# Kolkir/feature-point-cnn

Measured on AMD Instinct MI355X. Metric: frames/sec (VGA 640x480) SuperPoint fwd+NMS+descriptors, higher is better.
Workload: dtype f32

## Files before the change

feature-point-cnn_amd/_lib.py:

```python
import ctypes
import os
import subprocess

import torch

_DIR = os.path.dirname(os.path.abspath(__file__))
LIB_PATH = os.environ.get("FPC_LIB_PATH") or os.path.join(_DIR, "lib", "libfpc.so")
CSRC = os.path.join(_DIR, "csrc")

SYMBOLS = [
    "fpc_abi_version", "fpc_build_flags", "fpc_strerror", "fpc_last_hip_error", "fpc_default_config", "fpc_create",
    "fpc_destroy", "fpc_load_weights", "fpc_packed_size", "fpc_packed_device_ptr",
    "fpc_export_packed", "fpc_import_packed", "fpc_import_packed_device", "fpc_mark_weights_loaded", "fpc_set_stream", "fpc_upload_stream",
    "fpc_get_stream", "fpc_sync", "fpc_forward", "fpc_detect", "fpc_get_points", "fpc_results",
    "fpc_get_counts", "fpc_get_keypoints", "fpc_set_timing", "fpc_get_timings", "fpc_match", "fpc_first_within",
    "fpc_detect_u8", "fpc_u8_staging", "fpc_homography_adaptation", "fpc_detect_u8_resized",
    "fpc_sample_descriptors", "fpc_plan_hash", "fpc_broadcast_weights", "fpc_read_activation",
    "fpc_pack_layout_revision", "fpc_tile_choice", "fpc_check_guards", "fpc_stream_report", "fpc_output_range",
    "fpc_match_frames", "fpc_first_within_frames",
    "fpc_default_ransac_params", "fpc_ransac_homography", "fpc_homography_frames",
    "fpc_bank_create", "fpc_bank_destroy", "fpc_bank_get", "fpc_bank_store", "fpc_bank_store_rows", "fpc_bank_clear",
    "fpc_match_bank", "fpc_homography_bank", "fpc_bank_create_ex", "fpc_bank_format",
    "fpc_match_frames_guided", "fpc_match_bank_guided",
    "fpc_cell_order", "fpc_match_frames_guided_cells", "fpc_match_bank_guided_cells",
    "fpc_bank_topk_reserve", "fpc_match_bank_topk", "fpc_homography_bank_topk",
    "fpc_ransac_fundamental", "fpc_fundamental_frames", "fpc_fundamental_bank",
    "fpc_match_frames_guided_epipolar", "fpc_match_bank_guided_epipolar",
    "fpc_match_frames_guided_epipolar_cells", "fpc_match_bank_guided_epipolar_cells",
    "fpc_default_pose_params", "fpc_pose_fundamental", "fpc_pose_frames", "fpc_pose_bank",
    "fpc_default_pnp_params", "fpc_pnp_reserve", "fpc_bank_landmarks_reserve", "fpc_bank_store_landmarks",
    "fpc_bank_landmarks_get", "fpc_ransac_pnp", "fpc_pnp_frames", "fpc_pnp_bank",
]

ABI_VERSION = 4
PACK_LAYOUT_REVISION = 4

PLAN_FLAGS = {
    "no_fused_blocks": 1 << 0, "no_winograd": 1 << 1, "no_winograd_detector": 1 << 2, "no_winograd_layer_in1": 1 << 3,
    "no_xcd_order": 1 << 4, "no_fused_stem_pool": 1 << 5, "split_heads": 1 << 6, "nms_in_line": 1 << 7,
    "no_persistent_grid": 1 << 8, "layer1_tile_8x16": 1 << 9, "winograd_gen1": 1 << 10, "no_latency_tiles": 1 << 11,
    "nms_one_workgroup": 1 << 12, "no_fused_softmax": 1 << 13, "winograd_gen2": 1 << 14, "guard_zones": 1 << 15, "detector_gen1": 1 << 16, "heads_in_line": 1 << 17, "w36_one_wave": 1 << 18, "convt_phases": 1 << 19, "stem_round3": 1 << 20, "conv_round1": 1 << 21,
    "tiles_round5": 1 << 22,
}


class FpcConfig(ctypes.Structure):
    _fields_ = [("device", ctypes.c_int), ("height", ctypes.c_int), ("width", ctypes.c_int),
                ("max_batch", ctypes.c_int), ("cell", ctypes.c_int), ("nms_dist", ctypes.c_int),
                ("conf_thresh", ctypes.c_float), ("border_remove", ctypes.c_int),
                ("descriptor_enabled", ctypes.c_int), ("max_keypoints", ctypes.c_int),
                ("in_channels", ctypes.c_int), ("dtype", ctypes.c_int), ("arch", ctypes.c_int),
                ("num_streams", ctypes.c_int), ("plan_flags", ctypes.c_uint), ("nms_round_launches", ctypes.c_int),
                ("min_sub_batch", ctypes.c_int)]


class FpcTensor(ctypes.Structure):
    _fields_ = [("name", ctypes.c_char_p), ("data", ctypes.c_void_p), ("ndim", ctypes.c_int),
                ("shape", ctypes.c_int64 * 4)]


class FpcDeviceResults(ctypes.Structure):
    _fields_ = [("count", ctypes.c_void_p), ("n_candidates", ctypes.c_void_p), ("xy", ctypes.c_void_p),
                ("conf", ctypes.c_void_p), ("desc", ctypes.c_void_p), ("capacity", ctypes.c_int),
                ("desc_dim", ctypes.c_int)]


class FpcStreamReport(ctypes.Structure):
    _fields_ = [("n_streams", ctypes.c_int), ("slot", ctypes.c_int * 16), ("queue", ctypes.c_int * 16),
                ("probing", ctypes.c_int), ("hw_queues_found", ctypes.c_int), ("process_probe_rounds", ctypes.c_int),
                ("process_probe_launches", ctypes.c_int), ("process_inconclusive_rounds", ctypes.c_int),
                ("process_probe_ms", ctypes.c_float), ("create_probe_rounds", ctypes.c_int),
                ("create_placement_ms", ctypes.c_float), ("process_registered_streams", ctypes.c_int)]


class FpcRansacParams(ctypes.Structure):
# ... 170 lines not shown
```

feature-point-cnn_amd/csrc/block_mfma.h:

```cpp
#pragma once
#include "conv_mfma.h"

namespace fpc {

#ifdef FPC_DIAG
#define FPC_STAMP(i)                                                                     \
  if (a.stamps && threadIdx.x == 0) {                                                    \
    unsigned long long t_;                                                               \
    asm volatile("s_memtime %0\n\ts_waitcnt lgkmcnt(0)" : "=s"(t_)::"memory");            \
    a.stamps[(size_t)blockIdx.x * 8 + (i)] = t_;                                         \
  }
#define FPC_RSTAMP(i)                                                                    \
  if (a.stamps && threadIdx.x == 0) {                                                    \
    unsigned long long t_;                                                               \
    asm volatile("s_memrealtime %0\n\ts_waitcnt lgkmcnt(0)" : "=s"(t_)::"memory");        \
    a.stamps[(size_t)blockIdx.x * 8 + (i)] = t_;                                         \
  }
#else
#define FPC_STAMP(i)
#define FPC_RSTAMP(i)
#endif

struct BlockArgs {
  const float* x;
  int csx, nchunk;
  int H, W;
  const float4* w1;
  const float* b1;
  int tapoff4[9];
  const float4* w2;
  const float* b2;
  int k8_h, k8_x;
  float* out;
  int cso, Ho, Wo, tiles_x, tiles_y, nstore, frame0;
  unsigned x_bytes;
#ifdef FPC_DIAG
  unsigned long long* stamps;
#endif
};

template <int TH, int TW, int S, int KC, int WM, int WN, int MB, int NB, int CMIDP>
struct BlockCfg {
  using C1 = ConvCfg<TH, TW, S, 3, KC, WM, WN, MB, NB>;
  static constexpr int ROWH4 = CMIDP / 4 + 1;
  static constexpr int H_BYTES = C1::M * ROWH4 * 16;
  static constexpr int LDS_BYTES = C1::LDS_BYTES > H_BYTES ? C1::LDS_BYTES : H_BYTES;
  static_assert(CMIDP % 8 == 0 && CMIDP <= C1::N, "mid channels must fit the workgroup's N");
};

template <int TH, int TW, int S, int KC, int WM, int WN, int MB, int NB, int CMIDP>
__global__ __launch_bounds__(WM* WN * 64, 2) void block_mfma_kernel(const BlockArgs a) {
  using C = ConvCfg<TH, TW, S, 3, KC, WM, WN, MB, NB>;
  using BC = BlockCfg<TH, TW, S, KC, WM, WN, MB, NB, CMIDP>;
  constexpr int NT = C::NT, HW = C::HW, HH = C::HH, ROW4 = C::ROW4, K8 = KC / 8, KC4 = KC / 4;
  constexpr int NV = HH * HW * KC4, ITER = (NV + NT - 1) / NT, ROWH4 = BC::ROWH4, NBT = WN * NB;
  extern __shared__ float4 lds4[];

  const int tid = threadIdx.x, lane = tid & 63, wave = tid >> 6;
  const int wm = wave / WN, wn = wave % WN;
  const int half = lane >> 5, l31 = lane & 31;
  const int tiles = a.tiles_x * a.tiles_y;
  const int bidx = fpc_xcd_tile_index();
  const int bl = bidx / tiles;
  const int b = a.frame0 + bl;
  const int t = bidx - bl * tiles;
  const int ty = t / a.tiles_x, tx = t - ty * a.tiles_x;

  FPC_STAMP(0)
#ifdef FPC_DIAG
  if (a.stamps && threadIdx.x == 0) {
    a.stamps[(size_t)blockIdx.x * 8 + 6] = __builtin_amdgcn_s_getreg(63492);
    a.stamps[(size_t)blockIdx.x * 8 + 7] = __builtin_amdgcn_s_getreg((31 << 11) | 20);
  }
#endif
  int abase[MB];
#pragma unroll
  for (int mb = 0; mb < MB; ++mb) {
    int m = (wm * MB + mb) * 32 + l31;
    m = m < TH * TW ? m : TH * TW - 1;
    const int py = m / TW, px = m - py * TW;
    abase[mb] = ((py * S) * HW + px * S) * ROW4 + half;
  }
  constexpr int stepstride = NBT * 64;
  const __amdgpu_buffer_rsrc_t wrsrc = __builtin_amdgcn_make_buffer_rsrc(
      const_cast<float4*>(a.w1), 0, (int)((unsigned)(a.nchunk * 9 * K8 + 2) * (unsigned)(stepstride * 16)), 0x00020000);
  const int wlane = ((wn * NB) * 64 + lane) * 16;
  int wstep = 0;
  auto wfrag = [&](int nb) {
    typedef float f32x4w __attribute__((ext_vector_type(4)));
    const f32x4w r = __builtin_bit_cast(f32x4w, __builtin_amdgcn_raw_buffer_load_b128(wrsrc, wlane + nb * 1024, wstep, 0));
    return make_float4(r.x, r.y, r.z, r.w);
  };

  const int iy0 = ty * TH * S - 1, ix0 = tx * TW * S - 1;
  typedef float f32x4v __attribute__((ext_vector_type(4)));
  f32x4v stage[ITER];
  const __amdgpu_buffer_rsrc_t xrsrc = __builtin_amdgcn_make_buffer_rsrc(const_cast<float*>(a.x), 0, (int)a.x_bytes, 0x00020000);
  const unsigned xbase = (unsigned)((b * a.H + iy0) * a.W + ix0) * (unsigned)(a.csx * 4);
  auto load_chunk = [&](int chunk) {
    const int wlim = chunk < a.nchunk ? a.W : 0;
#pragma unroll
    for (int i = 0; i < ITER; ++i) {
      const int e = tid + i * NT;
      const int pix = e / KC4, c4 = e - pix * KC4;
      const int hy = pix / HW, hx = pix - hy * HW;
      const int iy = iy0 + hy, ix = ix0 + hx;
      const bool ok = ((unsigned)iy < (unsigned)a.H) & ((unsigned)ix < (unsigned)wlim) & (hy < HH);
      unsigned off = xbase + (unsigned)(((hy * a.W + hx) * a.csx + chunk * KC + c4 * 4) * 4);
      asm volatile("" : "+v"(off));
      stage[i] = __builtin_bit_cast(f32x4v, __builtin_amdgcn_raw_buffer_load_b128(xrsrc, (int)(ok ? off : 0xfffffff0u), 0, 0));
    }
  };
  auto store_chunk = [&]() {
#pragma unroll
    for (int i = 0; i < ITER; ++i) {
      const int e = tid + i * NT;
      int pix = e / KC4, c4 = e - pix * KC4;
      if (NV % NT != 0) {
        const bool in = e < NV;
        pix = in ? pix : HH * HW - 1;
        c4 = in ? c4 : KC4;
      }
      *reinterpret_cast<f32x4v*>(&lds4[pix * ROW4 + c4]) = stage[i];
    }
  };

  f32x16 acc[MB][NB];
#pragma unroll
  for (int mb = 0; mb < MB; ++mb)
#pragma unroll
    for (int nb = 0; nb < NB; ++nb)
#pragma unroll
      for (int r = 0; r < 16; ++r) acc[mb][nb][r] = 0.f;

  load_chunk(0);
  float4 b0[NB], b1[NB];
#pragma unroll
  for (int nb = 0; nb < NB; ++nb) b0[nb] = wfrag(nb);
  wstep += stepstride * 16;
#pragma unroll
// ... 181 lines not shown
        const int e = tid + i * NT;
        const int m = e / C4, c4 = e - m * C4;
        const int py = m / TW, px = m - py * TW;
        const int y = oyb + py, x = oxb + px;
        const bool ok = (NE % NT == 0 || e < NE) && y < a.Ho && x < a.Wo;
        idv[i] = *reinterpret_cast<const float4*>(a.x + (ok ? ((size_t)(b * a.Ho + y) * a.Wo + x) * a.csx + c4 * 4 : 0));
      }
    }
#pragma unroll
    for (int i = 0; i < EIT; ++i) {
      const int e = tid + i * NT;
      const int m = e / C4, c4 = e - m * C4;
      const int py = m / TW, px = m - py * TW;
      const int y = oyb + py, x = oxb + px;
      if ((NE % NT == 0 || e < NE) && y < a.Ho && x < a.Wo) {
        float4 v = lds4[m * ROWH4 + c4];
        if (ident) {
          v.x += idv[i].x;
          v.y += idv[i].y;
          v.z += idv[i].z;
          v.w += idv[i].w;
        }
        v.x = v.x > 0.f ? v.x : 0.f;
        v.y = v.y > 0.f ? v.y : 0.f;
        v.z = v.z > 0.f ? v.z : 0.f;
        v.w = v.w > 0.f ? v.w : 0.f;
        *reinterpret_cast<float4*>(a.out + ((size_t)(b * a.Ho + y) * a.Wo + x) * a.cso + c4 * 4) = v;
      }
    }
  }
  FPC_STAMP(5)
}


}
```

feature-point-cnn_amd/csrc/fpc_api.hip:

```cpp
#include <hip/hip_runtime.h>

#include <dlfcn.h>

#include <algorithm>
#include <cmath>
#include <cstdio>
#include <cstdlib>
#include <cstring>
#include <memory>
#include <mutex>
#include <chrono>
#include <string>
#include <vector>

#include "../../include/fpc.h"
#include "block_mfma.h"
#include "block_bf16.h"
#include "convt_bf16.h"
#include "block_x3.h"
#include "stem_bf16.h"
#include "wblock_mfma.h"
#include "wblock16_mfma.h"
#include "wblock36_mfma.h"
#include "wblock36p_mfma.h"
// ... 126 lines not shown
enum BKind {
#define X(name, ...) BK_##name,
  FPC_BLOCK_KINDS(X)
#undef X
      BK_COUNT
};

struct BKindInfo {
  const char* name;
  const char* symbol;
  int TH, TW, S, KC, WM, WN, MB, NB, CMIDP;
  int lds_bytes;
  const void* fn;
  void (*launch)(const BlockArgs&, dim3, hipStream_t);
};

#define X(name, TH, TW, S, KC, WM, WN, MB, NB, CMIDP)                                                     \
  static void launchb_##name(const BlockArgs& a, dim3 grid, hipStream_t st) {                             \
    using BC = BlockCfg<TH, TW, S, KC, WM, WN, MB, NB, CMIDP>;                                            \
    hipLaunchKernelGGL((block_mfma_kernel<TH, TW, S, KC, WM, WN, MB, NB, CMIDP>), grid, dim3(WM* WN * 64), \
                       BC::LDS_BYTES, st, a);                                                             \
  }
FPC_BLOCK_KINDS(X)
#undef X

static const BKindInfo g_bkinds[BK_COUNT] = {
#define X(name, TH, TW, S, KC, WM, WN, MB, NB, CMIDP)                                                      \
  {#name, "block_mfma_kernel<" #TH ", " #TW ", " #S ", " #KC ", " #WM ", " #WN ", " #MB ", " #NB ", " #CMIDP ">", \
   TH, TW, S, KC, WM, WN, MB, NB, CMIDP, BlockCfg<TH, TW, S, KC, WM, WN, MB, NB, CMIDP>::LDS_BYTES,         \
   (const void*)block_mfma_kernel<TH, TW, S, KC, WM, WN, MB, NB, CMIDP>, launchb_##name},
    FPC_BLOCK_KINDS(X)
#undef X
};

#define FPC_WBLOCK_KINDS(X)     \
  X(W816_K32_C64, 32, 2, 64)    \
  X(W816_K32_C128, 32, 4, 128)  \
  X(W816_K32_C72, 32, 3, 72)    \
  X(W816_K24_C72, 24, 3, 72)
#define FPC_W16_KINDS(X) \
  X(W16_C64, 4, 8)       \
  X(W16_C128, 8, 8)      \
  X(W16_C128H, 8, 4)
#define FPC_W36_KINDS(X) \
  X(W36_C64_4x4, 1, 4, 4)  \
  X(W36_C64_2x8, 1, 2, 8)  \
  X(W36_C128_4x4, 2, 4, 4) \
  X(W36_C128_2x8, 2, 2, 8)

#define FPC_W36P_KINDS(X) \
  X(W36P_C64_4x4, 4, 4)   \
  X(W36P_C64_2x8, 2, 8)

#define FPC_W36PD_KINDS(X) \
  X(W36PD_C65_4x4, 4, 4)   \
  X(W36PD_C65_2x8, 2, 8)

#define FPC_W36D_KINDS(X) \
  X(W36_C65_4x4, 4, 4)    \
  X(W36_C65_2x8, 2, 8)

#define FPC_W36S_KINDS(X) \
  X(W36S_C128_4x4, 2, 4, 4)
#define FPC_W36PC_KINDS(X) \
  X(W36PC_C64_8x2, 8, 2)

// ... 243 lines not shown
  BlockArgs bargs{};
  WKind wkind = WK_COUNT;
  int hash_bkind = -1, hash_wkind = -1;
  WBlockArgs wargs{};
  FKind fkind = FK_COUNT;
  BlockBfArgs fargs{};
  int phase = -1;
  int when = 0;
  bool shadow = false;
  bool wconv = false;
  int n0 = 0;
  bool plain_conv = false;
  bool lean = false;
  int ksize = 0;
  const float* pin = nullptr;
  float* pout = nullptr;
  int pH = 0, pW = 0, pC = 0;
  std::string prefix;
  int cin = 0, cout = 0;
  int grid_y = 1, grid_z = 1;
  double flops_per_frame = 0;
  double mfma_flops_per_frame = 0;
  bool fused_softmax_capable = false;
  double bytes_per_frame = 0;
  bool descriptor_branch = false;
};

struct Timing {
  hipEvent_t start, stop;
  int op;
  int frames;
  int wkind = -1;
  double mfma_flops = -1.0;
};

}

using namespace fpc;

struct fpc_ctx {
  fpc_config cfg{};
  int H = 0, W = 0, B = 0, Hc = 0, Wc = 0;
  bool vgg = false;
  int D = 128;
  std::vector<float*> vbuf;
  size_t vconv0_off = 0;
  bool bf16 = false;
  bool split = false;
  bool split_f16 = false;
  int lgcs = 72;
  int cin = 3;
  int cap = 0, sort_cap = 0;
  hipStream_t stream = nullptr;
  bool own_stream = false;
  hipStream_t upload = nullptr;
  bool queue_probe = true;
  int probe_rounds = 0;
  double placement_ms = 0.0;
  std::vector<std::pair<hipStream_t, int>> caller_stream_memo;
  std::vector<hipStream_t> aux;
  std::vector<hipEvent_t> ev_join;
  std::vector<hipStream_t> side;
  std::vector<hipEvent_t> ev_enc, ev_det;
  bool nms_aside = true;
  bool split_heads = false;
  hipEvent_t ev_fork = nullptr;
  int min_sub = 8;
  int num_cus = 256;
  int fkind_blocks_per_cu[64] = {};
  int persist_min_tiles = 1;
  bool xcd_order = true;
  int nms_passes = 2;
  bool fuse_softmax = true;
  bool convt_fused = true;
  bool logits_valid = false;
  bool nms_one_workgroup = false;
  int nms_g = 0;
  bool fuse_stem_pool = true;
  bool conv_lean = true;
  bool stem_lean = true;
  bool stem2 = false;
  bool layer1_t816 = false;
#ifdef FPC_DIAG
  unsigned long long* diag_stamps = nullptr;
  int diag_n = 0;
#endif
  bool winograd_in1 = true;
  bool winograd_det = true;
  int w36_cus = 0;
  bool tiles_round6 = true;
  bool w36_paired = true;
  bool winograd_det_gen3 = true;
  bool winograd = true;
  bool latency_tiles = true;
  int winograd_gen = 3;
  bool fuse_blocks = true;
  bool weights_loaded = false;
  bool plan_error = false;

  char* slab = nullptr;
  size_t slab_bytes = 0;
  bool guard_zones = false;
  std::vector<std::pair<size_t, size_t>> guards;
  float *stem_out, *x0, *h4, *x1, *x2, *h8, *x3, *cat, *dh, *dproj, *d0, *lg;
  float *h16, *y16a, *y16b, *lo_h, *lo0, *desc_map, *desc_in_nhwc;
  float* prob;
  uint32_t *nmsmap, *cand;
  int32_t *ncand, *count, *xy, *status;
  float* rowmax = nullptr;
  uint32_t* range = nullptr;
  float *conf, *desc_out;
  unsigned long long* sort_scratch;
  int32_t* nms_aux = nullptr;
  unsigned long long *rowbest, *colbest;
  float* mf_norms = nullptr;
  unsigned long long *mf_top2 = nullptr, *mf_colbest = nullptr;
  float4* hf_pairs = nullptr;
  int32_t *hf_row = nullptr, *hf_np = nullptr;
  unsigned long long* hf_best = nullptr;
  int32_t *mgc_perm_q = nullptr, *mgc_perm_t = nullptr;
  int4* mgc_box = nullptr;
  char* bank_slab = nullptr;
// ... 1671 lines not shown
      default: break;
    }
    if (rc != FPC_OK) return rc;
  }
  return FPC_OK;
}

static hipEvent_t next_event(fpc_ctx* c) {
  if (c->events_used == c->event_pool.size()) {
    hipEvent_t e;
    hipEventCreate(&e);
    c->event_pool.push_back(e);
  }
  return c->event_pool[c->events_used++];
}

struct Sub {
  int f0, n;
  bool small = false;
  bool fuse_softmax = false;
  hipStream_t st;
  hipStream_t side = nullptr;
  hipEvent_t ev_enc = nullptr, ev_det = nullptr;
};

struct LaunchTimer {
  fpc_ctx* c;
  int op;
  hipStream_t st;
  int frames;
  hipEvent_t s{}, e{};
  int wkind = -1;
  double mfma_flops = -1.0;
  LaunchTimer(fpc_ctx* c_, int op_, hipStream_t st_, int frames_) : c(c_), op(op_), st(st_), frames(frames_) {
    if (c->timing) {
      s = next_event(c);
      e = next_event(c);
      hipEventRecord(s, st);
    }
  }
  ~LaunchTimer() {
    if (c->timing) {
      hipEventRecord(e, st);
      c->timings.push_back({s, e, op, frames, wkind, mfma_flops});
    }
  }
};

static int op_index(const fpc_ctx* c, OpType t) {
  for (size_t i = 0; i < c->ops.size(); ++i)
    if (c->ops[i].type == t) return (int)i;
  return -1;
}

template <typename Args>
static void diag_stamp(fpc_ctx* c, const Op& op, Args& a, int tiles) {
#ifdef FPC_DIAG
  a.stamps = nullptr;
  if (const char* e = getenv("FPC_STAMP_OP"))
    if (op.name.find(e) != std::string::npos) {
      if (!c->diag_stamps) hipHostMalloc((void**)&c->diag_stamps, (size_t)65536 * 8 * sizeof(unsigned long long));
      memset(c->diag_stamps, 0, (size_t)65536 * 8 * sizeof(unsigned long long));
      a.stamps = c->diag_stamps;
      c->diag_n = tiles;
    }
#endif
}

enum StemKind { STEM_PLAIN, STEM_POOL, STEM_POOL2, STEM_X3, STEM_X3_F16, STEM_BF16 };
static StemKind stem_kind(const fpc_ctx* c) {
  if (!(c->fuse_stem_pool || c->cin == 1 || c->bf16)) return STEM_PLAIN;
  if (c->split_f16) return STEM_X3_F16;
  if (c->bf16) return STEM_BF16;
  if (c->split) return STEM_X3;
  return c->stem2 ? STEM_POOL2 : STEM_POOL;
}

// ... 89 lines not shown
    const WKind sk = c->tiles_round6 ? w36_stacked_kind(op.wkind) : WK_COUNT;
    double mf = 0.0;
    for (int g0 = 0; g0 < n; g0 += fpl) {
      const int gn = std::min(fpl, n - g0);
      a.frame0 = 0;
      a.x = x0 + (size_t)(f0 + g0) * Hf * a.W * a.csx;
      a.out = o0 + (size_t)(f0 + g0) * Hf * a.W * a.cso;
      a.x_bytes = (unsigned)((unsigned long long)gn * Hf * a.W * a.csx * sizeof(float));
      const int srows = w36_stacked_rows(Hf, a.W, gn, sk, tx_f * ty_f);
      const WKind lk = srows ? sk : op.wkind;
      a.H = srows ? gn * Hf : Hf;
      a.frame_h = srows ? Hf : 0;
      a.tiles_x = srows ? (a.W + g_wkinds[sk].TW - 1) / g_wkinds[sk].TW : tx_f;
      a.tiles_y = srows ? srows : ty_f;
      a.total = srows ? a.tiles_x * srows : tx_f * ty_f * gn;
      if (srows) t.wkind = sk;
      mf += srows ? wkind_mfma_flops(g_wkinds[sk], a.total, a.nchunk, a.k8_h + a.k8_x) : op.mfma_flops_per_frame * gn;
      const int cus_cap = c->w36_cus > 0 ? std::min(c->num_cus, c->w36_cus) : c->num_cus;
      const int cus8 = std::max(1, cus_cap / 8 / std::max(1, op.grid_y)), per_xcd = (a.total + 7) / 8;
      const int rounds = (per_xcd + cus8 - 1) / cus8;
      const int grid3 = 8 * std::min(cus8, (per_xcd + rounds - 1) / rounds);
      g_wkinds[lk].launch(a, dim3(std::min(a.total, grid3), op.grid_y), sb.st);
    }
    if (t.wkind >= 0) t.mfma_flops = mf;
    return;
  }
  g_wkinds[op.wkind].launch(a, dim3(std::min(a.total, grid), op.grid_y), sb.st);
}

static void launch_block(fpc_ctx* c, const Op& op, int i, const Sub& sb) {
  LaunchTimer t(c, i, sb.st, sb.n);
  BlockArgs a = op.bargs;
  a.frame0 = sb.f0;
  diag_stamp(c, op, a, a.tiles_x * a.tiles_y * sb.n);
  g_bkinds[op.bkind].launch(a, dim3(a.tiles_x * a.tiles_y * sb.n), sb.st);
}

static void launch_fblock(fpc_ctx* c, const Op& op, int i, const Sub& sb) {
  const int n = sb.n, f0 = sb.f0;
  LaunchTimer t(c, i, sb.st, n);
  BlockBfArgs a = op.fargs;
  a.frame0 = f0;
  a.range_flag = c->split_f16 ? c->status + 1 : nullptr;
  diag_stamp(c, op, a, a.tiles_x * a.tiles_y * n);
  if (g_fkinds[op.fkind].planes != 1) {
    g_fkinds[op.fkind].launch(a, dim3(a.tiles_x * a.tiles_y * n), sb.st);
    return;
  }
  a.total_tiles = a.tiles_x * a.tiles_y * n;
  if (sb.fuse_softmax && op.fused_softmax_capable) {
    const size_t HW = (size_t)c->H * c->W;
    hipMemsetAsync(c->ncand + f0, 0, sizeof(int32_t) * n, sb.st);
    a.softmax = 1;
    a.thresh = c->cfg.conf_thresh;
    a.nmsmap = c->nmsmap + f0 * HW;
    a.cand = c->cand + f0 * HW;
    a.ncand = c->ncand + f0;
  }
  const int g = std::min((a.total_tiles + 7) / 8 * 8, std::max(8, c->fkind_blocks_per_cu[op.fkind] * c->num_cus / op.grid_y / 8 * 8));
  g_fkinds[op.fkind].launch(a, dim3(g, op.grid_y), sb.st);
}

static void launch_conv(fpc_ctx* c, const Op& op, int i, const Sub& sb) {
  LaunchTimer t(c, i, sb.st, sb.n);
  ConvArgs a = op.args;
  a.frame0 = sb.f0;
// ... 222 lines not shown
    case FPC_E_MISSING_KEY: return "checkpoint entry missing or of the wrong shape (see fpc_last_hip_error)";
    case FPC_E_CAPACITY: return "caller buffer too small";
    case FPC_E_NOT_CONVERGED: return "NMS round limit hit";
    case FPC_E_RANGE: return "value outside fp16's range in FPC_F32_SPLIT_F16 mode (use FPC_F32_SPLIT or FPC_F32)";
    case FPC_E_NONFINITE: return "a frame of the call holds a NaN or Inf pixel (see fpc_last_hip_error for which)";
    default: return "unknown error";
  }
}

const char* fpc_last_hip_error(void) { return g_hip_err.c_str(); }

int fpc_default_config(fpc_config* cfg) {
  if (!cfg) return FPC_E_INVALID;
  memset(cfg, 0, sizeof(*cfg));
  cfg->device = 0;
  cfg->height = 480;
  cfg->width = 640;
  cfg->max_batch = 1;
  cfg->cell = 8;
  cfg->nms_dist = 4;
  cfg->conf_thresh = 0.015f;
  cfg->border_remove = 4;
  cfg->descriptor_enabled = 1;
  cfg->max_keypoints = 0;
  return FPC_OK;
}

enum { SLOT_MAIN = 0, SLOT_AUX = 1, SLOT_SIDE = 100, SLOT_UPLOAD = 200 };

static int prepare_kernels(fpc_ctx* c, const fpc_config* cfg) {
  for (int k = 0; k < K_COUNT; ++k)
    HIPCHECK(hipFuncSetAttribute(g_kinds[k].fn, hipFuncAttributeMaxDynamicSharedMemorySize, g_kinds[k].lds_bytes));
  for (const LeanKindInfo& l : g_lean_kinds) HIPCHECK(hipFuncSetAttribute(l.fn, hipFuncAttributeMaxDynamicSharedMemorySize, l.lds_bytes));
  for (int k = 0; k < WK_COUNT; ++k)
    HIPCHECK(hipFuncSetAttribute(g_wkinds[k].fn, hipFuncAttributeMaxDynamicSharedMemorySize, g_wkinds[k].lds_bytes));
  for (int k = 0; k < BK_COUNT; ++k)
    HIPCHECK(hipFuncSetAttribute(g_bkinds[k].fn, hipFuncAttributeMaxDynamicSharedMemorySize, g_bkinds[k].lds_bytes));
  static_assert(FK_COUNT <= 64, "fpc_ctx::fkind_blocks_per_cu");
  for (int k = 0; k < FK_COUNT; ++k) {
    HIPCHECK(hipFuncSetAttribute(g_fkinds[k].fn, hipFuncAttributeMaxDynamicSharedMemorySize, g_fkinds[k].lds_bytes));
    int nb = 0;
    HIPCHECK(hipOccupancyMaxActiveBlocksPerMultiprocessor(&nb, g_fkinds[k].fn, g_fkinds[k].WM * g_fkinds[k].WN * 64, g_fkinds[k].lds_bytes));
    c->fkind_blocks_per_cu[k] = std::max(1, nb);
#ifdef FPC_DIAG
    hipFuncAttributes fa{};
    hipFuncGetAttributes(&fa, g_fkinds[k].fn);
    fprintf(stderr, "[diag] %s: lds %d B, regs %d, scratch %zu, occupancy %d blocks/CU\n", g_fkinds[k].name, g_fkinds[k].lds_bytes, fa.numRegs, fa.localSizeBytes, nb);
#endif
  }
  HIPCHECK(hipFuncSetAttribute((const void*)softmax_d2s_kernel<false>, hipFuncAttributeMaxDynamicSharedMemorySize,
                               12 * cfg->width * (int)sizeof(float)));
  HIPCHECK(hipFuncSetAttribute((const void*)softmax_d2s_kernel<true>, hipFuncAttributeMaxDynamicSharedMemorySize,
                               12 * cfg->width * (int)sizeof(float)));
  HIPCHECK(hipFuncSetAttribute((const void*)stem_bf16_kernel<1>, hipFuncAttributeMaxDynamicSharedMemorySize, StemB2Cfg<1>::LDS_BYTES));
  HIPCHECK(hipFuncSetAttribute((const void*)stem_bf16_kernel<3>, hipFuncAttributeMaxDynamicSharedMemorySize, StemB2Cfg<3>::LDS_BYTES));
  HIPCHECK(hipFuncSetAttribute((const void*)nms_sort_kernel, hipFuncAttributeMaxDynamicSharedMemorySize,
                               NMS_LDS_KEYS * (int)sizeof(unsigned long long)));
#ifdef FPC_DIAG
  for (int k = 0; k < BK_COUNT; ++k) {
    int nb = -1;
    hipOccupancyMaxActiveBlocksPerMultiprocessor(&nb, g_bkinds[k].fn, g_bkinds[k].WM * g_bkinds[k].WN * 64, g_bkinds[k].lds_bytes);
    hipFuncAttributes fa{};
    hipFuncGetAttributes(&fa, g_bkinds[k].fn);
    fprintf(stderr, "[diag] %s: lds %d B, regs %d, static lds %zu, occupancy %d blocks/CU\n", g_bkinds[k].name, g_bkinds[k].lds_bytes, fa.numRegs, fa.sharedSizeBytes, nb);
  }
  for (int k = 0; k < K_COUNT; ++k) {
// ... 43 lines not shown
  c->D = c->vgg ? 256 : 128;
  c->bf16 = cfg->dtype == FPC_BF16;
  c->split = cfg->dtype == FPC_F32_SPLIT || cfg->dtype == FPC_F32_SPLIT_F16;
  c->split_f16 = cfg->dtype == FPC_F32_SPLIT_F16;
  c->lgcs = (c->bf16 || c->split) ? 80 : 72;
  const int r1 = cfg->nms_dist + 1;
  const int worst = ((c->H + r1 - 1) / r1) * ((c->W + r1 - 1) / r1);
  c->cap = cfg->max_keypoints > 0 ? cfg->max_keypoints : worst;
  c->sort_cap = 1;
  while (c->sort_cap < worst) c->sort_cap <<= 1;
  {
    const int prc = prepare_kernels(c.get(), cfg);
    if (prc != FPC_OK) return prc;
  }
  const bool qprobe = qmap::probe_mode() != 0;
  c->queue_probe = qprobe;
  const auto create_t0 = std::chrono::steady_clock::now();
  std::unique_lock<std::mutex> queue_lock(qmap::state().mu);
  const int probe_rounds0 = qmap::state().dev[cfg->device].rounds;
  c->stream = qmap::acquire(cfg->device, c.get(), SLOT_MAIN, true, qprobe, true);
  if (!c->stream) { qmap::release_owner(c.get()); g_hip_err = "hipStreamCreateWithFlags"; return FPC_E_HIP; }
  c->own_stream = true;
  {
    int nsub = cfg->num_streams > 0 ? std::min(8, cfg->num_streams) : (c->split ? 3 : 2);
    const unsigned pf = cfg->plan_flags;
    c->fuse_blocks = !(pf & FPC_PLAN_NO_FUSED_BLOCKS);
    c->guard_zones = (pf & FPC_PLAN_GUARD_ZONES) != 0;
    if (const char* e = getenv("FPC_GUARD_ZONES")) c->guard_zones = atoi(e) != 0;
    c->winograd_det_gen3 = !(pf & FPC_PLAN_DETECTOR_GEN1);
    c->w36_paired = !(pf & FPC_PLAN_W36_ONE_WAVE);
    if (const char* e = getenv("FPC_W36_PAIRED")) c->w36_paired = atoi(e) != 0;
    c->tiles_round6 = !(pf & FPC_PLAN_TILES_ROUND5);
    if (const char* e = getenv("FPC_TILES_ROUND6")) c->tiles_round6 = atoi(e) != 0;
    if (const char* e = getenv("FPC_W36_CUS")) c->w36_cus = std::max(0, atoi(e));
    if (const char* e = getenv("FPC_WINOGRAD_DET_GEN")) c->winograd_det_gen3 = atoi(e) >= 3;
    c->winograd = !(pf & FPC_PLAN_NO_WINOGRAD);
    c->winograd_det = !(pf & FPC_PLAN_NO_WINOGRAD_DETECTOR);
    c->winograd_in1 = !(pf & FPC_PLAN_NO_WINOGRAD_LAYER_IN1);
    c->xcd_order = !(pf & FPC_PLAN_NO_XCD_ORDER);
    c->fuse_stem_pool = !(pf & FPC_PLAN_NO_FUSED_STEM_POOL);
    c->stem_lean = !(pf & FPC_PLAN_STEM_ROUND3);
    c->conv_lean = !(pf & FPC_PLAN_CONV_ROUND1);
    if (const char* e = getenv("FPC_CONV_LEAN")) c->conv_lean = atoi(e) != 0;
    if (const char* e = getenv("FPC_STEM_LEAN")) c->stem_lean = atoi(e) != 0;
    c->split_heads = (pf & FPC_PLAN_SPLIT_HEADS) != 0;
    if (pf & FPC_PLAN_NO_PERSISTENT_GRID) c->persist_min_tiles = 0;
    c->layer1_t816 = (pf & FPC_PLAN_LAYER1_TILE_8x16) != 0;
    c->winograd_gen = (pf & FPC_PLAN_WINOGRAD_GEN1) ? 1 : (pf & FPC_PLAN_WINOGRAD_GEN2) ? 2 : 3;
    if (const char* e = getenv("FPC_WINOGRAD_GEN")) c->winograd_gen = std::min(3, std::max(1, atoi(e)));
    c->latency_tiles = !(pf & FPC_PLAN_NO_LATENCY_TILES);
    if (const char* e = getenv("FPC_LATENCY_TILES")) c->latency_tiles = atoi(e) != 0;
    c->fuse_softmax = !(pf & FPC_PLAN_NO_FUSED_SOFTMAX);
    c->convt_fused = !(pf & FPC_PLAN_CONVT_PHASES);
    if (const char* e = getenv("FPC_CONVT_FUSED")) c->convt_fused = atoi(e) != 0;
    if (const char* e = getenv("FPC_FUSE_SOFTMAX")) c->fuse_softmax = atoi(e) != 0;
    c->nms_one_workgroup = (pf & FPC_PLAN_NMS_ONE_WORKGROUP) != 0;
    if (const char* e = getenv("FPC_NMS_CHUNKED")) c->nms_one_workgroup = atoi(e) == 0;
    if (cfg->min_sub_batch > 0) c->min_sub = cfg->min_sub_batch;
    if (cfg->nms_round_launches > 0) c->nms_passes = std::min(64, cfg->nms_round_launches);
    else if (cfg->nms_round_launches < 0) c->nms_passes = 0;
    if (const char* e = getenv("FPC_STREAMS")) nsub = std::max(1, std::min(8, atoi(e)));
    if (!(pf & FPC_PLAN_HEADS_IN_LINE) && nsub >= 2 && !c->vgg && !c->bf16 && !c->split) c->split_heads = true;
    if (const char* e = getenv("FPC_FUSE")) c->fuse_blocks = atoi(e) != 0;
    if (const char* e = getenv("FPC_WINOGRAD")) c->winograd = atoi(e) != 0;
    if (const char* e = getenv("FPC_XCD_ORDER")) c->xcd_order = atoi(e) != 0;
    if (const char* e = getenv("FPC_MIN_SUB")) c->min_sub = std::max(1, atoi(e));
// ... 146 lines not shown
  if (n != c->blob_floats * sizeof(float)) {
    g_hip_err = "packed weights: " + std::to_string(n) + " bytes, this context's plan packs " + std::to_string(c->blob_floats * sizeof(float));
    return FPC_E_INVALID;
  }
  HIPCHECK(hipSetDevice(c->cfg.device));
  uint32_t h[BLOB_HEADER_FLOATS];
  HIPCHECK(hipMemcpy(h, src_dev, sizeof(h), hipMemcpyDeviceToHost));
  if (!check_blob_header(c, h, &g_hip_err)) return FPC_E_INVALID;
  if (src_dev != (const void*)c->blob) {
    c->weights_loaded = false;
    HIPCHECK(hipMemcpy(c->blob, src_dev, n, hipMemcpyDeviceToDevice));
    HIPCHECK(hipDeviceSynchronize());
  }
  c->weights_loaded = true;
  return FPC_OK;
}

int fpc_mark_weights_loaded(fpc_ctx* c) {
  if (!c) return FPC_E_INVALID;
  uint32_t h[BLOB_HEADER_FLOATS];
  HIPCHECK(hipSetDevice(c->cfg.device));
  HIPCHECK(hipMemcpy(h, c->blob, sizeof(h), hipMemcpyDeviceToHost));
  if (!check_blob_header(c, h, &g_hip_err)) {
    c->weights_loaded = false;
    return FPC_E_INVALID;
  }
  c->weights_loaded = true;
  return FPC_OK;
}

uint64_t fpc_plan_hash(const fpc_ctx* c) { return c ? plan_hash(c) : 0; }

int fpc_tile_choice(int what, int H, int W, int frames, unsigned plan_flags) {
  const bool r6 = !(plan_flags & FPC_PLAN_TILES_ROUND5);
  if (H <= 0 || W <= 0 || frames <= 0) return FPC_E_INVALID;
  switch (what) {
    case 0: {
      const WKindInfo& k = g_wkinds[w36_kind(128, H, W)];
      return r6 ? w36_stacked_rows(H, W, frames, WK_W36S_C128_4x4, ((H + k.TH - 1) / k.TH) * ((W + k.TW - 1) / k.TW)) : 0;
    }
    case 1: { const WKindInfo& k = g_wkinds[w36_kind(64, H, W, true, r6)]; return 100 * k.TH + k.TW; }
    case 2: {
      const BKind k5 = BK_B320_s2_K32_C128, k6 = BK_B416_s2_K32_C128;
      const BKindInfo& k = g_bkinds[r6 && block_rows(k6, H, W) < block_rows(k5, H, W) ? k6 : k5];
      return 100 * k.TH + k.TW;
    }
  }
  return FPC_E_INVALID;
}

int fpc_check_guards(fpc_ctx* c, long long* bad_words) {
  if (!c || !bad_words) return FPC_E_INVALID;
  *bad_words = 0;
  if (!c->guard_zones || c->guards.empty()) return FPC_E_INVALID;
  HIPCHECK(hipSetDevice(c->cfg.device));
  HIPCHECK(hipDeviceSynchronize());
  unsigned long long* d = nullptr;
  HIPCHECK(hipMalloc((void**)&d, sizeof(*d)));
  {
    const hipError_t e0 = hipMemset(d, 0, sizeof(*d));
    if (e0 != hipSuccess) hipFree(d);
    HIPCHECK(e0);
  }
  count_zones(c, c->slab, c->guards, d);
  count_zones(c, c->bank_slab, c->bank_guards, d);
  count_zones(c, c->topk_slab, c->topk_guards, d);
  count_zones(c, c->pnp_slab, c->pnp_guards, d);
  count_zones(c, c->lm_slab, c->lm_guards, d);
  unsigned long long h = 0;
  const hipError_t e1 = hipStreamSynchronize(c->stream);
  const hipError_t e2 = hipMemcpy(&h, d, sizeof(h), hipMemcpyDeviceToHost);
  hipFree(d);
  HIPCHECK(e1);
  HIPCHECK(e2);
  *bad_words = (long long)h;
  return FPC_OK;
}

namespace {
// ... 1320 lines not shown
  if (desc) {
    if (!c->cfg.descriptor_enabled) return FPC_E_INVALID;
    HIPCHECK(hipMemcpy(desc, c->desc_out + (size_t)frame * c->cap * c->D, sizeof(float) * c->D * k, hipMemcpyDeviceToHost));
  }
  return k;
}

int fpc_set_timing(fpc_ctx* c, int enable) {
  if (!c) return FPC_E_INVALID;
  c->timing_every = enable > 0 ? enable : 0;
  c->timing_calls = 0;
  c->timing = enable != 0;
  c->timings.clear();
  c->events_used = 0;
  return FPC_OK;
}

int fpc_get_timings(fpc_ctx* c, int cap, const char** names, const char** kernels, float* ms, double* flops,
                    double* mfma_flops, double* bytes) {
  if (!c) return FPC_E_INVALID;
  const int n = (int)c->timings.size();
  for (int i = 0; i < n && i < cap; ++i) {
    const Timing& t = c->timings[i];
    float v = 0.f;
    if (hipEventElapsedTime(&v, t.start, t.stop) != hipSuccess) v = -1.f;
    const Op* op = t.op >= 0 ? &c->ops[t.op] : nullptr;
    if (names) names[i] = op ? op->name.c_str() : "?";
    if (kernels) {
      const char* k = "?";
      if (op) switch (op->type) {
          case OP_STEM: k = launch_stem(c, *op, t.op, nullptr, nullptr); break;
          case OP_POOL: k = "maxpool_kernel"; break;
          case OP_CONV: k = op->lean ? lean_kind(op->kind)->symbol : g_kinds[op->kind].symbol; break;
          case OP_BLOCK: k = g_bkinds[op->bkind].symbol; break;
          case OP_WBLOCK: k = g_wkinds[t.wkind >= 0 ? t.wkind : op->wkind].symbol; break;
          case OP_BF16: k = g_fkinds[op->fkind].symbol; break;
          case OP_SOFTMAX: k = "softmax_d2s_kernel"; break;
          case OP_NMS: k = c->nms_one_workgroup ? "nms_rounds_kernel+nms_sort_kernel" : "nms_rounds_kernel+nms_finish_kernel+nms_chunk_sort_kernel+nms_merge_kernel"; break;
          case OP_DESC: k = "descriptor16_kernel"; break;
          case OP_VCONV0: k = "vgg_conv0_kernel"; break;
          case OP_POOL2: k = "maxpool2_kernel"; break;
          case OP_L2NORM: k = "l2norm256_kernel"; break;
        }
      kernels[i] = k;
    }
    if (ms) ms[i] = v;
    if (flops) flops[i] = op ? op->flops_per_frame * t.frames : 0.0;
    if (mfma_flops) mfma_flops[i] = !op ? 0.0 : t.mfma_flops >= 0 ? t.mfma_flops : op->mfma_flops_per_frame * t.frames;
    if (bytes) bytes[i] = op ? op->bytes_per_frame * t.frames : 0.0;
  }
  return n;
}

}
```

include/fpc.h:

```cpp
#ifndef FPC_H
#define FPC_H

#include <stddef.h>
#include <stdint.h>

#ifdef __cplusplus
extern "C" {
#endif

#define FPC_ABI_VERSION 4
#define FPC_PACK_LAYOUT_REVISION 4

enum {
  FPC_OK = 0,
  FPC_E_INVALID = -1,
  FPC_E_NO_DEVICE = -2,
  FPC_E_HIP = -3,
  FPC_E_NO_WEIGHTS = -4,
  FPC_E_MISSING_KEY = -5,
  FPC_E_CAPACITY = -6,
  FPC_E_NOT_CONVERGED = -7,
  FPC_E_RANGE = -8,
  FPC_E_NONFINITE = -9
};
// ... 14 lines not shown
  int max_keypoints;
  int in_channels;
  int dtype;
  int arch;
  int num_streams;
  unsigned plan_flags;
  int nms_round_launches;
  int min_sub_batch;
} fpc_config;

enum {
  FPC_PLAN_NO_FUSED_BLOCKS = 1 << 0,
  FPC_PLAN_NO_WINOGRAD = 1 << 1,
  FPC_PLAN_NO_WINOGRAD_DETECTOR = 1 << 2,
  FPC_PLAN_NO_WINOGRAD_LAYER_IN1 = 1 << 3,
  FPC_PLAN_NO_XCD_ORDER = 1 << 4,
  FPC_PLAN_NO_FUSED_STEM_POOL = 1 << 5,
  FPC_PLAN_SPLIT_HEADS = 1 << 6,
  FPC_PLAN_NMS_IN_LINE = 1 << 7,
  FPC_PLAN_NO_PERSISTENT_GRID = 1 << 8,
  FPC_PLAN_LAYER1_TILE_8x16 = 1 << 9,
  FPC_PLAN_WINOGRAD_GEN1 = 1 << 10,
  FPC_PLAN_NO_LATENCY_TILES = 1 << 11,
  FPC_PLAN_NMS_ONE_WORKGROUP = 1 << 12,
  FPC_PLAN_NO_FUSED_SOFTMAX = 1 << 13,
  FPC_PLAN_WINOGRAD_GEN2 = 1 << 14,
  FPC_PLAN_HEADS_IN_LINE = 1 << 17,
  FPC_PLAN_DETECTOR_GEN1 = 1 << 16,
  FPC_PLAN_W36_ONE_WAVE = 1 << 18,
  FPC_PLAN_STEM_ROUND3 = 1 << 20,
  FPC_PLAN_CONV_ROUND1 = 1 << 21,
  FPC_PLAN_CONVT_PHASES = 1 << 19,
  FPC_PLAN_TILES_ROUND5 = 1 << 22,
  FPC_PLAN_GUARD_ZONES = 1 << 15
};

typedef struct fpc_tensor {
  const char* name;
  const float* data;
  int ndim;
  int64_t shape[4];
} fpc_tensor;

typedef struct fpc_device_results {
  const int32_t* count;
  const int32_t* n_candidates;
  const int32_t* xy;
  const float* conf;
  const float* desc;
  int capacity;
  int desc_dim;
} fpc_device_results;

typedef struct fpc_ctx fpc_ctx;

int fpc_abi_version(void);
const char* fpc_build_flags(void);
const char* fpc_strerror(int code);
const char* fpc_last_hip_error(void);

int fpc_default_config(fpc_config* cfg);

int fpc_create(fpc_ctx** out, const fpc_config* cfg);
void fpc_destroy(fpc_ctx* ctx);

int fpc_load_weights(fpc_ctx* ctx, const fpc_tensor* tensors, int n);
// ... 203 lines not shown
```

Before: 12410.

## Stack frames vertically in stride-2 fused block to cut tile-quantisation waste

Adds a stacked variant of the fused stride-2 MFMA block kernel that treats a batch of frames as one tall image. Row tiles may now straddle frame seams, and the halo loader inserts a zero row at each seam so no tile reads across frames. The stacked path is used only when it yields fewer padded output rows than per-frame tiling. It removes the partial-tile waste at the bottom of each frame, at the cost of an extra halo row, more index arithmetic and a new plan flag to keep the old tiling.

```diff
diff --git a/feature-point-cnn_amd/_lib.py b/feature-point-cnn_amd/_lib.py
--- a/feature-point-cnn_amd/_lib.py
+++ b/feature-point-cnn_amd/_lib.py
@@ -40,7 +40,7 @@
     "no_xcd_order": 1 << 4, "no_fused_stem_pool": 1 << 5, "split_heads": 1 << 6, "nms_in_line": 1 << 7,
     "no_persistent_grid": 1 << 8, "layer1_tile_8x16": 1 << 9, "winograd_gen1": 1 << 10, "no_latency_tiles": 1 << 11,
     "nms_one_workgroup": 1 << 12, "no_fused_softmax": 1 << 13, "winograd_gen2": 1 << 14, "guard_zones": 1 << 15, "detector_gen1": 1 << 16, "heads_in_line": 1 << 17, "w36_one_wave": 1 << 18, "convt_phases": 1 << 19, "stem_round3": 1 << 20, "conv_round1": 1 << 21,
-    "tiles_round5": 1 << 22,
+    "tiles_round5": 1 << 22, "tiles_round6": 1 << 23,
 }
 
 
diff --git a/feature-point-cnn_amd/csrc/block_mfma.h b/feature-point-cnn_amd/csrc/block_mfma.h
--- a/feature-point-cnn_amd/csrc/block_mfma.h
+++ b/feature-point-cnn_amd/csrc/block_mfma.h
@@ -37,22 +37,26 @@
 #ifdef FPC_DIAG
   unsigned long long* stamps;
 #endif
+  int frame_h;
 };
 
-template <int TH, int TW, int S, int KC, int WM, int WN, int MB, int NB, int CMIDP>
+template <int TH, int TW, int S, int KC, int WM, int WN, int MB, int NB, int CMIDP, bool STACK = false>
 struct BlockCfg {
   using C1 = ConvCfg<TH, TW, S, 3, KC, WM, WN, MB, NB>;
+  static constexpr int HHS = C1::HH + (STACK ? 1 : 0);
   static constexpr int ROWH4 = CMIDP / 4 + 1;
   static constexpr int H_BYTES = C1::M * ROWH4 * 16;
-  static constexpr int LDS_BYTES = C1::LDS_BYTES > H_BYTES ? C1::LDS_BYTES : H_BYTES;
+  static constexpr int HALO_BYTES = HHS * C1::HW * C1::ROW4 * 16;
+  static constexpr int LDS_BYTES = HALO_BYTES > H_BYTES ? HALO_BYTES : H_BYTES;
   static_assert(CMIDP % 8 == 0 && CMIDP <= C1::N, "mid channels must fit the workgroup's N");
+  static_assert(!STACK || S == 2, "the stacked walk is written for the stride-2 blocks");
 };
 
-template <int TH, int TW, int S, int KC, int WM, int WN, int MB, int NB, int CMIDP>
-__global__ __launch_bounds__(WM* WN * 64, 2) void block_mfma_kernel(const BlockArgs a) {
+template <int TH, int TW, int S, int KC, int WM, int WN, int MB, int NB, int CMIDP, bool STACK>
+__device__ __forceinline__ void block_mfma_body(const BlockArgs& a) {
   using C = ConvCfg<TH, TW, S, 3, KC, WM, WN, MB, NB>;
-  using BC = BlockCfg<TH, TW, S, KC, WM, WN, MB, NB, CMIDP>;
-  constexpr int NT = C::NT, HW = C::HW, HH = C::HH, ROW4 = C::ROW4, K8 = KC / 8, KC4 = KC / 4;
+  using BC = BlockCfg<TH, TW, S, KC, WM, WN, MB, NB, CMIDP, STACK>;
+  constexpr int NT = C::NT, HW = C::HW, HH = BC::HHS, ROW4 = C::ROW4, K8 = KC / 8, KC4 = KC / 4;
   constexpr int NV = HH * HW * KC4, ITER = (NV + NT - 1) / NT, ROWH4 = BC::ROWH4, NBT = WN * NB;
   extern __shared__ float4 lds4[];
 
@@ -65,6 +69,12 @@
   const int b = a.frame0 + bl;
   const int t = bidx - bl * tiles;
   const int ty = t / a.tiles_x, tx = t - ty * a.tiles_x;
+  int seam = TH, zrow = HH;
+  if constexpr (STACK) {
+    const int hof = a.frame_h / S, r = ty * TH % hof;
+    seam = r == 0 ? 0 : hof - r;
+    zrow = seam < TH ? S * seam + 1 : HH;
+  }
 
   FPC_STAMP(0)
 #ifdef FPC_DIAG
@@ -79,7 +89,7 @@
     int m = (wm * MB + mb) * 32 + l31;
     m = m < TH * TW ? m : TH * TW - 1;
     const int py = m / TW, px = m - py * TW;
-    abase[mb] = ((py * S) * HW + px * S) * ROW4 + half;
+    abase[mb] = ((py * S + (STACK && py >= seam ? 1 : 0)) * HW + px * S) * ROW4 + half;
   }
   constexpr int stepstride = NBT * 64;
   const __amdgpu_buffer_rsrc_t wrsrc = __builtin_amdgcn_make_buffer_rsrc(
@@ -103,9 +113,10 @@
     for (int i = 0; i < ITER; ++i) {
       const int e = tid + i * NT;
       const int pix = e / KC4, c4 = e - pix * KC4;
-      const int hy = pix / HW, hx = pix - hy * HW;
+      const int hl = pix / HW, hx = pix - hl * HW;
+      const int hy = STACK ? hl - (hl > zrow ? 1 : 0) : hl;
       const int iy = iy0 + hy, ix = ix0 + hx;
-      const bool ok = ((unsigned)iy < (unsigned)a.H) & ((unsigned)ix < (unsigned)wlim) & (hy < HH);
+      const bool ok = ((unsigned)iy < (unsigned)a.H) & ((unsigned)ix < (unsigned)wlim) & (hl < HH) & (!STACK || hl != zrow);
       unsigned off = xbase + (unsigned)(((hy * a.W + hx) * a.csx + chunk * KC + c4 * 4) * 4);
       asm volatile("" : "+v"(off));
       stage[i] = __builtin_bit_cast(f32x4v, __builtin_amdgcn_raw_buffer_load_b128(xrsrc, (int)(ok ? off : 0xfffffff0u), 0, 0));
@@ -353,5 +364,14 @@
   FPC_STAMP(5)
 }
 
-
+template <int TH, int TW, int S, int KC, int WM, int WN, int MB, int NB, int CMIDP>
+__global__ __launch_bounds__(WM* WN * 64, 2) void block_mfma_kernel(const BlockArgs a) {
+  block_mfma_body<TH, TW, S, KC, WM, WN, MB, NB, CMIDP, false>(a);
 }
+template <int TH, int TW, int S, int KC, int WM, int WN, int MB, int NB, int CMIDP>
+__global__ __launch_bounds__(WM* WN * 64, 2) void block_mfma_stacked_kernel(const BlockArgs a) {
+  block_mfma_body<TH, TW, S, KC, WM, WN, MB, NB, CMIDP, true>(a);
+}
+
+
+}
diff --git a/feature-point-cnn_amd/csrc/fpc_api.hip b/feature-point-cnn_amd/csrc/fpc_api.hip
--- a/feature-point-cnn_amd/csrc/fpc_api.hip
+++ b/feature-point-cnn_amd/csrc/fpc_api.hip
@@ -182,6 +182,46 @@
     FPC_BLOCK_KINDS(X)
 #undef X
 };
+
+#define FPC_BLOCK_STACKED_KINDS(X) \
+  X(B48_s2_K32_C256, B310_s2_K32_C256, 4, 8, 2, 32, 1, 4, 1, 2, 256)
+struct BlockStackedInfo {
+  BKind of;
+  const char* symbol;
+  int TH, TW, S, KC, M, N;
+  int lds_bytes;
+  const void* fn;
+  void (*launch)(const BlockArgs&, dim3, hipStream_t);
+};
+#define X(name, of, TH, TW, S, KC, WM, WN, MB, NB, CMIDP)                                                        \
+  static void launchbs_##name(const BlockArgs& a, dim3 grid, hipStream_t st) {                                   \
+    using BC = BlockCfg<TH, TW, S, KC, WM, WN, MB, NB, CMIDP, true>;                                             \
+    hipLaunchKernelGGL((block_mfma_stacked_kernel<TH, TW, S, KC, WM, WN, MB, NB, CMIDP>), grid, dim3(WM* WN * 64), \
+                       BC::LDS_BYTES, st, a);                                                                    \
+  }
+FPC_BLOCK_STACKED_KINDS(X)
+#undef X
+static const BlockStackedInfo g_block_stacked_kinds[] = {
+#define X(name, of, TH, TW, S, KC, WM, WN, MB, NB, CMIDP)                                                                 \
+  {BK_##of, "block_mfma_stacked_kernel<" #TH ", " #TW ", " #S ", " #KC ", " #WM ", " #WN ", " #MB ", " #NB ", " #CMIDP ">", \
+   TH, TW, S, KC, WM * MB * 32, WN * NB * 32, BlockCfg<TH, TW, S, KC, WM, WN, MB, NB, CMIDP, true>::LDS_BYTES,             \
+   (const void*)block_mfma_stacked_kernel<TH, TW, S, KC, WM, WN, MB, NB, CMIDP>, launchbs_##name},
+    FPC_BLOCK_STACKED_KINDS(X)
+#undef X
+};
+static const BlockStackedInfo* block_stacked_kind(BKind op_kind) {
+  const BKindInfo& k = g_bkinds[op_kind];
+  for (const BlockStackedInfo& l : g_block_stacked_kinds) {
+    const BKindInfo& o = g_bkinds[l.of];
+    if (k.KC == o.KC && k.WN * k.NB == o.WN * o.NB && k.S == o.S && k.CMIDP == o.CMIDP) return &l;
+  }
+  return nullptr;
+}
+static int block_stacked_rows(const BlockStackedInfo& s, int Ho, int Wo, int frames, long rows_now) {
+  if (frames < 2 || Ho < s.TH) return 0;
+  const int rows = (frames * Ho + s.TH - 1) / s.TH;
+  return (long)rows * ((Wo + s.TW - 1) / s.TW) * s.M < (long)frames * rows_now ? rows : 0;
+}
 
 #define FPC_WBLOCK_KINDS(X)     \
   X(W816_K32_C64, 32, 2, 64)    \
@@ -491,6 +531,7 @@
   int frames;
   int wkind = -1;
   double mfma_flops = -1.0;
+  const char* symbol = nullptr;
 };
 
 }
@@ -547,6 +588,7 @@
   bool winograd_in1 = true;
   bool winograd_det = true;
   int w36_cus = 0;
+  bool tiles_round7 = true;
   bool tiles_round6 = true;
   bool w36_paired = true;
   bool winograd_det_gen3 = true;
@@ -2284,6 +2326,7 @@
   hipEvent_t s{}, e{};
   int wkind = -1;
   double mfma_flops = -1.0;
+  const char* symbol = nullptr;
   LaunchTimer(fpc_ctx* c_, int op_, hipStream_t st_, int frames_) : c(c_), op(op_), st(st_), frames(frames_) {
     if (c->timing) {
       s = next_event(c);
@@ -2294,7 +2337,7 @@
   ~LaunchTimer() {
     if (c->timing) {
       hipEventRecord(e, st);
-      c->timings.push_back({s, e, op, frames, wkind, mfma_flops});
+      c->timings.push_back({s, e, op, frames, wkind, mfma_flops, symbol});
     }
   }
 };
@@ -2450,6 +2493,30 @@
   LaunchTimer t(c, i, sb.st, sb.n);
   BlockArgs a = op.bargs;
   a.frame0 = sb.f0;
+  const BlockStackedInfo* sk = c->tiles_round7 && !sb.small ? block_stacked_kind(op.bkind) : nullptr;
+  const unsigned long long sbytes = (unsigned long long)sb.n * a.H * a.W * a.csx * sizeof(float);
+  if (sk && a.H == sk->S * a.Ho && a.W == sk->S * a.Wo && sbytes < 0xffffff00ull) {
+    const int rows = block_stacked_rows(*sk, a.Ho, a.Wo, sb.n, block_rows(op.bkind, a.Ho, a.Wo));
+    if (rows) {
+      const int HWp = (sk->TW - 1) * sk->S + 3, ROW4 = sk->KC / 4 + 1;
+      for (int ky = 0; ky < 3; ++ky)
+        for (int kx = 0; kx < 3; ++kx) a.tapoff4[ky * 3 + kx] = (ky * HWp + kx) * ROW4;
+      a.x += (size_t)sb.f0 * a.H * a.W * a.csx;
+      a.out += (size_t)sb.f0 * a.Ho * a.Wo * a.cso;
+      a.x_bytes = (unsigned)sbytes;
+      a.frame0 = 0;
+      a.frame_h = a.H;
+      a.H *= sb.n;
+      a.Ho *= sb.n;
+      a.tiles_x = (a.Wo + sk->TW - 1) / sk->TW;
+      a.tiles_y = rows;
+      t.symbol = sk->symbol;
+      t.mfma_flops = 2.0 * a.tiles_x * rows * sk->M * (double)sk->N * ((double)a.nchunk * sk->KC * 9 + (a.k8_h + a.k8_x) * 8.0);
+      diag_stamp(c, op, a, a.tiles_x * rows);
+      sk->launch(a, dim3(a.tiles_x * rows), sb.st);
+      return;
+    }
+  }
   diag_stamp(c, op, a, a.tiles_x * a.tiles_y * sb.n);
   g_bkinds[op.bkind].launch(a, dim3(a.tiles_x * a.tiles_y * sb.n), sb.st);
 }
@@ -2738,6 +2805,7 @@
   for (int k = 0; k < K_COUNT; ++k)
     HIPCHECK(hipFuncSetAttribute(g_kinds[k].fn, hipFuncAttributeMaxDynamicSharedMemorySize, g_kinds[k].lds_bytes));
   for (const LeanKindInfo& l : g_lean_kinds) HIPCHECK(hipFuncSetAttribute(l.fn, hipFuncAttributeMaxDynamicSharedMemorySize, l.lds_bytes));
+  for (const BlockStackedInfo& l : g_block_stacked_kinds) HIPCHECK(hipFuncSetAttribute(l.fn, hipFuncAttributeMaxDynamicSharedMemorySize, l.lds_bytes));
   for (int k = 0; k < WK_COUNT; ++k)
     HIPCHECK(hipFuncSetAttribute(g_wkinds[k].fn, hipFuncAttributeMaxDynamicSharedMemorySize, g_wkinds[k].lds_bytes));
   for (int k = 0; k < BK_COUNT; ++k)
@@ -2847,6 +2915,9 @@
     if (const char* e = getenv("FPC_W36_PAIRED")) c->w36_paired = atoi(e) != 0;
     c->tiles_round6 = !(pf & FPC_PLAN_TILES_ROUND5);
     if (const char* e = getenv("FPC_TILES_ROUND6")) c->tiles_round6 = atoi(e) != 0;
+    c->tiles_round7 = !(pf & (FPC_PLAN_TILES_ROUND5 | FPC_PLAN_TILES_ROUND6));
+    if (const char* e = getenv("FPC_TILES_ROUND7")) c->tiles_round7 = atoi(e) != 0;
+    c->tiles_round7 = c->tiles_round7 && c->tiles_round6;
     if (const char* e = getenv("FPC_W36_CUS")) c->w36_cus = std::max(0, atoi(e));
     if (const char* e = getenv("FPC_WINOGRAD_DET_GEN")) c->winograd_det_gen3 = atoi(e) >= 3;
     c->winograd = !(pf & FPC_PLAN_NO_WINOGRAD);
@@ -3059,7 +3130,7 @@
 uint64_t fpc_plan_hash(const fpc_ctx* c) { return c ? plan_hash(c) : 0; }
 
 int fpc_tile_choice(int what, int H, int W, int frames, unsigned plan_flags) {
-  const bool r6 = !(plan_flags & FPC_PLAN_TILES_ROUND5);
+  const bool r6 = !(plan_flags & FPC_PLAN_TILES_ROUND5), r7 = r6 && !(plan_flags & FPC_PLAN_TILES_ROUND6);
   if (H <= 0 || W <= 0 || frames <= 0) return FPC_E_INVALID;
   switch (what) {
     case 0: {
@@ -3072,6 +3143,8 @@
       const BKindInfo& k = g_bkinds[r6 && block_rows(k6, H, W) < block_rows(k5, H, W) ? k6 : k5];
       return 100 * k.TH + k.TW;
     }
+    case 4:
+      return r7 ? block_stacked_rows(g_block_stacked_kinds[0], H, W, frames, block_rows(BK_B310_s2_K32_C256, H, W)) : 0;
   }
   return FPC_E_INVALID;
 }
@@ -4458,7 +4531,7 @@
           case OP_STEM: k = launch_stem(c, *op, t.op, nullptr, nullptr); break;
           case OP_POOL: k = "maxpool_kernel"; break;
           case OP_CONV: k = op->lean ? lean_kind(op->kind)->symbol : g_kinds[op->kind].symbol; break;
-          case OP_BLOCK: k = g_bkinds[op->bkind].symbol; break;
+          case OP_BLOCK: k = t.symbol ? t.symbol : g_bkinds[op->bkind].symbol; break;
           case OP_WBLOCK: k = g_wkinds[t.wkind >= 0 ? t.wkind : op->wkind].symbol; break;
           case OP_BF16: k = g_fkinds[op->fkind].symbol; break;
           case OP_SOFTMAX: k = "softmax_d2s_kernel"; break;
diff --git a/include/fpc.h b/include/fpc.h
--- a/include/fpc.h
+++ b/include/fpc.h
@@ -70,6 +70,7 @@
   FPC_PLAN_CONV_ROUND1 = 1 << 21,
   FPC_PLAN_CONVT_PHASES = 1 << 19,
   FPC_PLAN_TILES_ROUND5 = 1 << 22,
+  FPC_PLAN_TILES_ROUND6 = 1 << 23,
   FPC_PLAN_GUARD_ZONES = 1 << 15
 };
 
```

After: 12420 (median of 6 runs). No clear change (+0.1%).
